# Beryl2000/SE-UNet-AirSeg

Hardware: AMD Instinct MI355X
Metric: voxels/sec SE-UNet fwd+bwd, 128^3 patch (higher is better)
Workload: dtype bf16

## Files before the change

### se-unet-airseg_amd/csrc/abi.cpp

```cpp
#include "seunet_common.h"
#include "epilogue.h"
#include "volume.h"
#include "wgrad.h"
#include "../../include/seunet_hip.h"

using namespace seunet;

static inline Dims D(seunet_dims d) { return Dims{d.n, d.d, d.h, d.w}; }
static inline hipStream_t S(seunet_stream_t s) { return reinterpret_cast<hipStream_t>(s); }

static int make_src(int nsrc, const void* const* src, const int* src_c, SrcList& l) {
  SEUNET_CHECK(nsrc >= 1 && nsrc <= 3 && src && src_c, "bad source list");
  l = SrcList{};
  l.n = nsrc;
  for (int i = 0; i < nsrc; ++i) { l.ptr[i] = src[i]; l.C[i] = src_c[i]; }
  return 0;
}

namespace seunet { extern unsigned long long* g_conv_debug; }

extern "C" {

int seunet_debug_set_buffer(void* p) { seunet::g_conv_debug = reinterpret_cast<unsigned long long*>(p); return 0; }
int seunet_debug_upsample2_form(int dtype, int c, seunet_dims dims, int backward) { return upsample2_form(dtype, c, D(dims), backward != 0); }
// ... 236 lines not shown
                         seunet_stream_t s) {
  SEUNET_CHECK(side && out && scale >= 1, "side_upsample: bad argument");
  return launch_side_upsample(side, c, scale, out, c_total, c_off, D(low), S(s));
}

int seunet_head_fwd(const float* const* level_maps, int nlevels, const float* bias, float* pred, seunet_dims d, seunet_stream_t s) {
  SEUNET_CHECK(level_maps && bias && pred, "head_fwd: null tensor");
  return launch_head_fwd(level_maps, nlevels, bias, pred, D(d), S(s));
}
size_t seunet_head_bwd_tmp_floats(seunet_dims d) { return head_bwd_tmp_floats(D(d)); }
int seunet_head_bwd(const float* g_pred, float* const* g_levels, int nlevels, float* tmp, float* g_bias, seunet_dims d,
                    seunet_stream_t s) {
  SEUNET_CHECK(g_pred && g_levels && tmp, "head_bwd: null tensor");
  return launch_head_bwd(g_pred, g_levels, nlevels, tmp, g_bias, D(d), S(s));
}

int seunet_loss_partial_floats(void) { return loss_partials() * SEUNET_LOSS_NSUMS; }
int seunet_loss_sums(const float* pred, int apply_sigmoid, const float* target, const float* weight, const float* skel,
                     long long n, float* partial, double* sums, int terms, seunet_stream_t s) {
  SEUNET_CHECK(pred && target && partial && sums && n >= 1, "loss_sums: bad argument");
  SEUNET_CHECK(terms >= 0 && terms <= 7, "loss_sums: terms=%d is not a mask of SEUNET_LOSS_DICE | _GUL | _ATR", terms);
  return launch_loss_sums(pred, apply_sigmoid, target, weight, skel, n, partial, sums, S(s), terms);
}
int seunet_loss_value(const double* sums0, double c_dice0, double c_gul0, double c_atr0, const double* sums1, double c_dice1,
                      double c_gul1, double c_atr1, float* value, seunet_stream_t s) {
  SEUNET_CHECK(sums0 && value, "loss_value: null argument");
  return launch_loss_value(sums0, c_dice0, c_gul0, c_atr0, sums1, c_dice1, c_gul1, c_atr1, value, S(s));
}
int seunet_loss_grad(const float* pred, int apply_sigmoid, const float* target, const float* weight, const float* skel,
                     long long n, const double* sums, float c_dice, float c_gul, float c_atr, float g_scale,
// ... 413 lines not shown
```

### se-unet-airseg_amd/csrc/heads.hip

```cpp
#include "seunet_common.h"
#include "trilinear.h"

namespace seunet {

__global__ void side_upsample_kernel(const float* __restrict__ side, int C, int scale,
                                     float* __restrict__ out, int c_total, int c_off, int D, int H, int W,
                                     long long total) {
  const int Do = D * scale, Ho = H * scale, Wo = W * scale;
  const float rz = ac_scale(D, Do), ry = ac_scale(H, Ho), rx = ac_scale(W, Wo);
  const long long Vo = (long long)Do * Ho * Wo;
  for (long long i = blockIdx.x * (long long)blockDim.x + threadIdx.x; i < total;
       i += (long long)gridDim.x * blockDim.x) {
    long long r = i;
    const int xo = (int)(r % Wo); r /= Wo;
    const int yo = (int)(r % Ho); r /= Ho;
    const int zo = (int)(r % Do);
    const long long n = r / Do;
    int z0, z1, y0, y1, x0, x1; float lz, ly, lx;
    ac_src(zo, rz, D, z0, z1, lz);
    ac_src(yo, ry, H, y0, y1, ly);
    ac_src(xo, rx, W, x0, x1, lx);
    for (int c = 0; c < C; ++c) {
      float acc = 0.f;
#pragma unroll
// ... 46 lines not shown
      const float w00 = (1.f - lz) * (1.f - ly), w01 = (1.f - lz) * ly, w10 = lz * (1.f - ly), w11 = lz * ly;
      const float rx = ac_scale(Wl, W);
#pragma unroll
      for (int k = 0; k < 4; ++k) {
        int x0, x1; float lx;
        ac_src(4 * xq + k, rx, Wl, x0, x1, lx);
        const float a0 = w00 * r00[x0] + w01 * r01[x0] + w10 * r10[x0] + w11 * r11[x0];
        const float a1 = w00 * r00[x1] + w01 * r01[x1] + w10 * r10[x1] + w11 * r11[x1];
        acc[k] += (1.f - lx) * a0 + lx * a1;
      }
    }
    *reinterpret_cast<float4*>(pred + o) = make_float4(acc[0], acc[1], acc[2], acc[3]);
  }
}
constexpr int HF_RPW = 4;
__global__ void __launch_bounds__(256)
head_fwd_rows_kernel(HeadLevels lv, const float* __restrict__ bias, float* __restrict__ pred, int D, int H, int W) {
  extern __shared__ float hrow[];
  const int wv = __builtin_amdgcn_readfirstlane(threadIdx.x >> 6), lane = threadIdx.x & 63;
  const int per_row = (W >> 1) + (W >> 2) + (W >> 3);
  float* const rb = hrow + wv * HF_RPW * per_row;
  const float b0 = bias[0];
  const int ybl = (H + 4 * HF_RPW - 1) / (4 * HF_RPW);
  const int yb = blockIdx.x % ybl, zo = (blockIdx.x / ybl) % D, n = blockIdx.x / (ybl * D);
  const int ybase = (yb * 4 + wv) * HF_RPW;
  float2 v0[HF_RPW];
#pragma unroll
  for (int r = 0; r < HF_RPW; ++r) {
    const int yo = ybase + r < H ? ybase + r : H - 1;
    v0[r] = (lv.map[0] && 2 * lane < W) ? *reinterpret_cast<const float2*>(lv.map[0] + (((long long)n * D + zo) * H + yo) * W + 2 * lane)
                                        : make_float2(0.f, 0.f);
  }
  int tx0[3][2], tx1[3][2]; float tlx[3][2];
#pragma unroll
  for (int l = 1; l < 4; ++l)
#pragma unroll
    for (int k = 0; k < 2; ++k) ac_src(2 * lane + k, ac_scale(W >> l, W), W >> l, tx0[l - 1][k], tx1[l - 1][k], tlx[l - 1][k]);
#pragma unroll
  for (int l = 1; l < 4; ++l) {
    if (!lv.map[l]) continue;
    const int Dl = D >> l, Hl = H >> l, Wl = W >> l;
    int z0, z1; float lz;
    ac_src(zo, ac_scale(Dl, D), Dl, z0, z1, lz);
    const float* m = lv.map[l] + (long long)n * Dl * Hl * Wl;
    const int lbase = (l > 1 ? (W >> 1) : 0) + (l > 2 ? (W >> 2) : 0);
#pragma unroll
    for (int r = 0; r < HF_RPW; ++r) {
      const int yo = ybase + r < H ? ybase + r : H - 1;
      int y0, y1; float ly;
      ac_src(yo, ac_scale(Hl, H), Hl, y0, y1, ly);
      const float* r00 = m + (z0 * Hl + y0) * Wl;
      const float* r01 = m + (z0 * Hl + y1) * Wl;
      const float* r10 = m + (z1 * Hl + y0) * Wl;
      const float* r11 = m + (z1 * Hl + y1) * Wl;
      const float w00 = (1.f - lz) * (1.f - ly), w01 = (1.f - lz) * ly, w10 = lz * (1.f - ly), w11 = lz * ly;
      for (int xc = lane; xc < Wl; xc += 64)
        rb[r * per_row + lbase + xc] = w00 * r00[xc] + w01 * r01[xc] + w10 * r10[xc] + w11 * r11[xc];
    }
  }
  __builtin_amdgcn_wave_barrier();
#pragma unroll
  for (int r = 0; r < HF_RPW; ++r) {
    const int yo = ybase + r;
    if (yo >= H) break;
    const long long orow = (((long long)n * D + zo) * H + yo) * W;
    for (int x = 2 * lane; x < W; x += 128) {
      float acc[2] = {b0, b0};
      if (lv.map[0]) {
        const float2 v = x < 128 ? v0[r] : *reinterpret_cast<const float2*>(lv.map[0] + orow + x);
        acc[0] += v.x; acc[1] += v.y;
      }
      int lb = r * per_row;
// ... 3 lines not shown
        const int Wl = W >> l;
#pragma unroll
        for (int k = 0; k < 2; ++k) {
          int x0 = tx0[l - 1][k], x1 = tx1[l - 1][k]; float lx = tlx[l - 1][k];
          if (x >= 128) ac_src(x + k, ac_scale(Wl, W), Wl, x0, x1, lx);
          acc[k] += (1.f - lx) * rb[lb + x0] + lx * rb[lb + x1];
        }
        lb += Wl;
      }
      *reinterpret_cast<float2*>(pred + orow + x) = make_float2(acc[0], acc[1]);
    }
  }
}

constexpr int HB_ROWS = 32, HB_K = 24, HB_PAD = 24, HB_KA = 8;
__global__ void __launch_bounds__(256)
head_bwd_x_multi_kernel(const float* __restrict__ g, float* __restrict__ t1a, float* __restrict__ t1b, float* __restrict__ t1c,
                        int nl, int W, long long rows, double* __restrict__ bias_part) {
  extern __shared__ float hsm[];
  const int RW = W + HB_PAD;
  float* tab = hsm + 4 * RW;
  const int wv = threadIdx.x >> 6, lane = threadIdx.x & 63;
  const long long row0 = (long long)blockIdx.x * HB_ROWS;
  constexpr int RPW = HB_ROWS / 4;
  const bool pf = W <= 256;
  float pre[RPW][4];
  if (pf) {
#pragma unroll
    for (int j = 0; j < RPW; ++j) {
      const long long row = row0 + wv + 4 * j;
#pragma unroll
      for (int k = 0; k < 4; ++k) {
        const int x = lane + 64 * k;
        pre[j][k] = (row < rows && x < W) ? g[row * W + x] : 0.f;
      }
    }
  }
  float* const outs[3] = {t1a, t1b, t1c};
  int ebase[4] = {0, 0, W >> 1, (W >> 1) + (W >> 2)};
  const int nent = (nl > 1 ? W >> 1 : 0) + (nl > 2 ? W >> 2 : 0) + (nl > 3 ? W >> 3 : 0);
  for (int e = threadIdx.x; e < nent; e += 256) {
    const int l = e < ebase[2] ? 1 : (e < ebase[3] ? 2 : 3);
    const int i = e - ebase[l], Wl = W >> l;
    const float rs = ac_scale(Wl, W);
    int lo, hi;
    ac_range(i, rs, W, lo, hi);
    float* t = tab + e * (HB_K + 2);
    int cnt = 0, first = lo;
    bool started = false;
    for (int o = lo; o <= hi; ++o) {
      const float w = ac_weight(o, i, rs, Wl);
      if (!started && w == 0.f) { first = o + 1; continue; }
      started = true;
      if (cnt < HB_K) t[2 + cnt] = w;
      ++cnt;
    }
    t[0] = __int_as_float(first);
    t[1] = __int_as_float(cnt < HB_K ? cnt : HB_K);
  }
  for (int i = threadIdx.x; i < 4 * HB_PAD; i += 256) hsm[(i / HB_PAD) * RW + W + i % HB_PAD] = 0.f;
  __syncthreads();
  const int e0 = lane, e1 = lane + 64;
  float wa[HB_KA], wb[HB_K];
  int fa = 0, fb = 0, ca = 0, cb = 0;
  {
    if (e0 < nent) { const float* t = tab + e0 * (HB_K + 2); fa = __float_as_int(t[0]); ca = __float_as_int(t[1]); }
    if (e1 < nent) { const float* t = tab + e1 * (HB_K + 2); fb = __float_as_int(t[0]); cb = __float_as_int(t[1]); }
#pragma unroll
    for (int k = 0; k < HB_KA; ++k) wa[k] = (e0 < nent && k < ca) ? tab[e0 * (HB_K + 2) + 2 + k] : 0.f;
#pragma unroll
    for (int k = 0; k < HB_K; ++k) wb[k] = (e1 < nent && k < cb) ? tab[e1 * (HB_K + 2) + 2 + k] : 0.f;
  }
  const bool fast = nent <= 128 && __all(ca <= HB_KA && cb <= HB_K && fa + HB_KA <= RW && fb + HB_K <= RW);
  int ka = 0, kb = 0;
#pragma unroll
  for (int off = 32; off >= 1; off >>= 1) { ca = max(ca, shfl_xor_settled(ca, off)); cb = max(cb, shfl_xor_settled(cb, off)); }
  ka = (ca + 3) & ~3; kb = (cb + 3) & ~3;
  const int la = e0 < ebase[2] ? 1 : (e0 < ebase[3] ? 2 : 3), lb = e1 < ebase[2] ? 1 : (e1 < ebase[3] ? 2 : 3);
  float* const outa = e0 < nent ? (la == 1 ? t1a : (la == 2 ? t1b : t1c)) : nullptr;
  float* const outb = e1 < nent ? (lb == 1 ? t1a : (lb == 2 ? t1b : t1c)) : nullptr;
  const int cola = e0 - ebase[la], colb = e1 - ebase[lb], wla = W >> la, wlb = W >> lb;
  double sum = 0.0;
#pragma unroll
  for (int j = 0; j < RPW; ++j) {
    const int rr = wv + 4 * j;
    const long long row = row0 + rr;
    if (row >= rows) break;
    float* rb = hsm + wv * RW;
    if (pf) {
#pragma unroll
      for (int k = 0; k < 4; ++k) {
        const int x = lane + 64 * k;
        if (x < W) { rb[x] = pre[j][k]; sum += (double)pre[j][k]; }
      }
    } else {
      for (int x = lane; x < W; x += 64) { const float v = g[row * W + x]; rb[x] = v; sum += (double)v; }
    }
    __builtin_amdgcn_wave_barrier();
    if (fast) {
      float a0 = 0.f, a1 = 0.f;
#pragma unroll
      for (int k = 0; k < HB_KA; ++k)
        if (k < ka) a0 += wa[k] * rb[fa + k];
#pragma unroll
      for (int k = 0; k < HB_K; ++k)
        if (k < kb) a1 += wb[k] * rb[fb + k];
      if (outa) outa[row * wla + cola] = a0;
      if (outb) outb[row * wlb + colb] = a1;
      __builtin_amdgcn_wave_barrier();
      continue;
    }
    for (int e = lane; e < nent; e += 64) {
      const int l = e < ebase[2] ? 1 : (e < ebase[3] ? 2 : 3);
      float* out = outs[l - 1];
      if (out == nullptr) continue;
      const float* t = tab + e * (HB_K + 2);
      const int first = __float_as_int(t[0]), cnt = __float_as_int(t[1]);
      float acc = 0.f;
      for (int k = 0; k < cnt; k += 4) {
        float w[4], v[4];
#pragma unroll
        for (int j = 0; j < 4; ++j) {
          const bool in = k + j < cnt;
          w[j] = in ? t[2 + k + j] : 0.f;
          v[j] = in ? rb[first + k + j] : 0.f;
        }
#pragma unroll
        for (int j = 0; j < 4; ++j)
          if (w[j] != 0.f) acc += w[j] * v[j];
      }
      out[row * (W >> l) + (e - ebase[l])] = acc;
    }
    __builtin_amdgcn_wave_barrier();
  }
  if (bias_part != nullptr) {
#pragma unroll
    for (int off = 32; off >= 1; off >>= 1) sum += shfl_xor_settled(sum, off);
    __shared__ double wsum[4];
    if (lane == 0) wsum[wv] = sum;
    __syncthreads();
    if (threadIdx.x == 0) bias_part[blockIdx.x] = ((wsum[0] + wsum[1]) + wsum[2]) + wsum[3];
  }
}

__global__ void __launch_bounds__(1024) sum_stage2_wide_kernel(const double* __restrict__ partial, int n, float* __restrict__ out) {
  double s = 0.0;
  for (int i = threadIdx.x; i < n; i += 1024) s += partial[i];
#pragma unroll
  for (int off = 32; off >= 1; off >>= 1) s += shfl_xor_settled(s, off);
  __shared__ double w[16];
  if ((threadIdx.x & 63) == 0) w[threadIdx.x >> 6] = s;
  __syncthreads();
  if (threadIdx.x == 0) {
    double t = 0.0;
    for (int k = 0; k < 16; ++k) t += w[k];
    out[0] = (float)t;
// ... 14 lines not shown
  if (threadIdx.x == 0) {
    double t = 0.0;
    for (int k = 0; k < 16; ++k) t += w[k];
    out[0] = (float)t;
  }
}

int launch_side_upsample(const float* side, int C, int scale, float* out, int c_total, int c_off, Dims dl,
                         hipStream_t s) {
  const long long total = (long long)dl.N * dl.vox() * scale * scale * scale;
  side_upsample_kernel<<<grid_for(total), 256, 0, s>>>(side, C, scale, out, c_total, c_off, dl.D, dl.H, dl.W, total);
  SEUNET_LAUNCH_CHECK();
  return 0;
}

int launch_head_fwd(const float* const* level_maps, int nlevels, const float* bias, float* pred, Dims d0,
                    hipStream_t s) {
  SEUNET_CHECK(nlevels >= 1 && nlevels <= 4, "head: nlevels=%d out of range", nlevels);
  HeadLevels lv;
  for (int l = 0; l < 4; ++l) lv.map[l] = l < nlevels ? level_maps[l] : nullptr;
  for (int l = 1; l < nlevels; ++l)
    SEUNET_CHECK((d0.D >> l) >= 1 && (d0.H >> l) >= 1 && (d0.W >> l) >= 1, "head: volume too small for level %d", l);
  SEUNET_CHECK(d0.W % 4 == 0, "head: W=%d must be a multiple of 4", d0.W);
  if (d0.W % 8 == 0 && d0.W <= 2048 && (long long)d0.D * d0.H * d0.W < (1ll << 31)) {
    const size_t lds = (size_t)4 * HF_RPW * ((d0.W >> 1) + (d0.W >> 2) + (d0.W >> 3)) * sizeof(float);
    const int ybl = (d0.H + 4 * HF_RPW - 1) / (4 * HF_RPW);
    head_fwd_rows_kernel<<<d0.N * d0.D * ybl, 256, lds, s>>>(lv, bias, pred, d0.D, d0.H, d0.W);
  } else {
    const long long total4 = (long long)d0.N * d0.vox() / 4;
    head_fwd_kernel<<<grid_for(total4), 256, 0, s>>>(lv, bias, pred, d0.D, d0.H, d0.W, total4);
  }
  SEUNET_LAUNCH_CHECK();
  return 0;
}

struct AxisJob { const float* in; float* out; int I, O; long long inner, total; };
struct AxisJobs { AxisJob j[3]; int njobs; const double* bias_part; int bias_n; float* g_bias; };
__global__ void __launch_bounds__(256) up_transpose_axis_multi_kernel(AxisJobs jobs) {
  if ((int)blockIdx.y >= jobs.njobs) {
    if (blockIdx.x == 0) sum_stage2_wide_by_256(jobs.bias_part, jobs.bias_n, jobs.g_bias);
    return;
  }
  const AxisJob jb = jobs.j[blockIdx.y];
  if (jb.total == 0) return;
  const float rs = ac_scale(jb.I, jb.O);
  const unsigned inner = (unsigned)jb.inner, I = (unsigned)jb.I, total = (unsigned)jb.total;
  for (unsigned idx = blockIdx.x * blockDim.x + threadIdx.x; idx < total; idx += gridDim.x * blockDim.x) {
    const unsigned q = idx / inner;
    const unsigned in_i = idx - q * inner;
    const unsigned outer = q / I;
    const int i = (int)(q - outer * I);
    int lo, hi;
    ac_range(i, rs, jb.O, lo, hi);
    float acc = 0.f;
    for (int o = lo; o <= hi; o += 4) {
// ... 15 lines not shown
static HeadBwdLayout head_bwd_layout(Dims d0, int nlevels) {
  HeadBwdLayout m{};
  const long long rows = (long long)d0.N * d0.D * d0.H, V = rows * d0.W;
  long long off = 0, off2 = V - V / 8;
  for (int l = 1; l < nlevels; ++l) {
    m.t1[l] = off;
    off += rows * (d0.W >> l);
    m.t2[l] = off2;
    off2 += (long long)d0.N * d0.D * (d0.H >> l) * (d0.W >> l);
  }
  m.part = (V + V / 2 + 64 + 1) & ~1ll;
  m.total = V + V / 2 + 64 + 2 * ((rows + HB_ROWS - 1) / HB_ROWS + 64);
  return m;
}
size_t head_bwd_tmp_floats(Dims d0) { return (size_t)head_bwd_layout(d0, 4).total; }
int launch_head_bwd(const float* g_pred, float* const* g_levels, int nlevels, float* tmp, float* g_bias,
                    Dims d0, hipStream_t s) {
  SEUNET_CHECK(nlevels >= 1 && nlevels <= 4, "head: nlevels=%d out of range", nlevels);
  const long long rows = (long long)d0.N * d0.D * d0.H;
  const long long V = rows * d0.W;
  const HeadBwdLayout m = head_bwd_layout(d0, nlevels);
  float* t1[4] = {nullptr, nullptr, nullptr, nullptr};
  float* t2[4] = {nullptr, nullptr, nullptr, nullptr};
  for (int l = 1; l < nlevels; ++l) {
    if (g_levels[l]) t1[l] = tmp + m.t1[l];
    t2[l] = tmp + m.t2[l];
  }
  double* part = reinterpret_cast<double*>(tmp + m.part);
  const int nblk = (int)((rows + HB_ROWS - 1) / HB_ROWS);
  SEUNET_CHECK(d0.W <= 1024, "head_bwd: W=%d too large", d0.W);
  SEUNET_CHECK(V / 2 < (1ll << 31), "head_bwd: %lld voxels per call exceed the 32-bit index range of the axis passes", V);
  const size_t lds = ((size_t)4 * (d0.W + HB_PAD) + (size_t)(d0.W - (d0.W >> 3)) * (HB_K + 2)) * sizeof(float);
  head_bwd_x_multi_kernel<<<nblk, 256, lds, s>>>(g_pred, t1[1], t1[2], t1[3], nlevels, d0.W, rows, g_bias ? part : nullptr);
  AxisJobs jy{}, jz{};
  long long max_y = 0, max_z = 0;
  int njobs = 0;
  for (int l = 1; l < nlevels; ++l) {
    if (!g_levels[l]) continue;
    const int Dl = d0.D >> l, Hl = d0.H >> l, Wl = d0.W >> l;
    const long long ty = (long long)d0.N * d0.D * Hl * Wl, tz = (long long)d0.N * Dl * Hl * Wl;
    jy.j[njobs] = AxisJob{t1[l], t2[l], Hl, d0.H, (long long)Wl, ty};
    jz.j[njobs] = AxisJob{t2[l], g_levels[l], Dl, d0.D, (long long)Hl * Wl, tz};
    max_y = ty > max_y ? ty : max_y;
    max_z = tz > max_z ? tz : max_z;
    ++njobs;
  }
  jy.njobs = jz.njobs = njobs;
  if (njobs) {
    if (g_bias) { jy.bias_part = part; jy.bias_n = nblk; jy.g_bias = g_bias; }
    up_transpose_axis_multi_kernel<<<dim3((unsigned)grid_for(max_y), (unsigned)njobs + (g_bias ? 1 : 0)), 256, 0, s>>>(jy);
    up_transpose_axis_multi_kernel<<<dim3((unsigned)grid_for(max_z), (unsigned)njobs), 256, 0, s>>>(jz);
  } else if (g_bias) {
    sum_stage2_wide_kernel<<<1, 1024, 0, s>>>(part, nblk, g_bias);
  }
  SEUNET_LAUNCH_CHECK();
  return 0;
}

}
```

### se-unet-airseg_amd/csrc/net.cpp

```cpp
#include "seunet_common.h"
#include "epilogue.h"
#include "wgrad.h"
#include "../../include/seunet_hip.h"

#include <algorithm>
#include <cstdio>
#include <cstring>
#include <string>
#include <vector>

namespace seunet {

ConvKernel wgrad_kernel(int dtype, int taps, int dil, const SrcList& x, int cin_logical, int cout, Dims d, long long src_dist) {
  if (taps == 1) {
    const int combos = cdiv(cin_logical, 32) * cdiv(cout, 32);
    const long long nv = (long long)d.N * d.vox();
    const bool pays = combos >= 16 || (combos >= 8 && nv >= 500000);
    return pays && wgrad_1x1_supported(dtype, x, cin_logical, cout) ? ConvKernel::Wgrad1x1 : ConvKernel::Tiled;
  }
  const bool fine = d.W >= 32 && (long long)d.D * d.H * d.W >= 48LL * 48 * 48;
  const bool pays = fine || dil == 2 || cin_logical >= 256;
  return pays && wgrad_march_supported(dtype, taps, dil, x, cin_logical, cout, d, src_dist) ? ConvKernel::March : ConvKernel::Tiled;
}

// ... 500 lines not shown
    const int t = c.o.src[0];
    mark("pool_fwd:", c.o.name);
    return launch_maxpool_fwd(p.d.dtype, at(p.feat[t]), p.C[t], at(p.feat[c.o.dst]), p.dims_of(t), s);
  }

  int up_forward(const Op& c) {
    const int t = c.o.src[0];
    mark("up_fwd:", c.o.name);
    return launch_upsample2_fwd(p.d.dtype, at(p.feat[t]), p.C[t], at(p.feat[c.o.dst]), p.dims_of(t), s);
  }

  int heads_forward(float* pred0, float* pred1) {
    float* const pred[2] = {pred0, pred1};
    const Dims d1{1, p.dims[0].D, p.dims[0].H, p.dims[0].W};
    mark("head_fwd");
    for (int h = 0; h < 2; ++h) {
      if (pred[h] == nullptr) continue;
      const int nl = 4 - h;
      if (p.d.n_classes > 1) {
        if (int e = per_sample_class(p.lvl[h], 0, nl, [&](float* const* lm, size_t nc) {
              return launch_head_fwd(lm, nl, par(kG.head_b[h]) + nc % p.d.n_classes, pred[h] + nc * d1.vox(), d1, s);
            })) return e;
      } else {
        const float* lm[4] = {fat(p.lvl[h][0]), fat(p.lvl[h][1]), fat(p.lvl[h][2]), fat(p.lvl[h][3])};
        if (int e = launch_head_fwd(lm, nl, par(kG.head_b[h]), pred[h], p.dims[0], s)) return e;
      }
    }
    mark("outside");
    return 0;
  }

  int forward(const float* x, const float* drop1, const float* drop2, float* pred0, float* pred1) {
    skip_enc_head = pred0 == nullptr;
    drops[0] = drop1; drops[1] = drop2;
    if (int e = pack_all_weights(false)) return e;
    mark("pack_input");
    if (int e = launch_pack_input(p.d.dtype, x, p.d.in_channel, at(p.feat[T_X0]), p.dims[0], s)) return e;
    for (int i = 0; i < kNumOps; ++i) {
      const Op c = op(i);
      const OpKind k = c.o.kind;
      if (int e = k == OP_GATED ? gated_forward(c) : k == OP_CAT ? cat_forward(c) : k == OP_POOL ? pool_forward(c) : up_forward(c))
// ... 38 lines not shown
    gd.n = x.n;
    for (int k = 0; k < x.n; ++k) {
      const int t = o.src[k];
      gd.C[k] = p.C[t];
      gd.ptr[k] = is_input(t) ? nullptr : at(p.grad[t]);
      gd.acc[k] = (!is_input(t) && written[t]) ? 1 : 0;
      if (!is_input(t)) written[t] = true;
    }
    mark("dgrad:", o.name);
    return run_conv(r.dgrad, r.taps, o.dil, gsrc, r.cout, par(c.i, P_CONV1_W), 1, at(r.wp_d), nullptr, gd, nullptr, c.dm);
  }

  int heads_backward() {
    const Dims d1{1, p.dims[0].D, p.dims[0].H, p.dims[0].W};
    mark("head_bwd");
    for (int h = 0; h < 2; ++h) {
      const int nl = 4 - h;
      float* gb = grads[kG.head_b[h]];
      if (p.d.n_classes > 1) {
        if (int e = per_sample_class(p.glvl[h], 1, nl, [&](float* const* gl, size_t nc) {
              return launch_head_bwd(g_pred[h] + nc * d1.vox(), gl, nl, fat(p.head_tmp), fat(p.cls_bias) + nc, d1, s);
            })) return e;
        if (gb)
          if (int e = launch_class_bias_grad(fat(p.cls_bias), p.d.batch, p.d.n_classes, gb, s)) return e;
      } else {
        float* gl[4] = {nullptr, fat(p.glvl[h][1]), fat(p.glvl[h][2]), nl == 4 ? fat(p.glvl[h][3]) : nullptr};
        if (int e = launch_head_bwd(g_pred[h], gl, nl, fat(p.head_tmp), gb, p.dims[0], s)) return e;
      }
    }
    return 0;
  }

  int gated_backward(const Op& c) {
    const OpDesc& o = c.o;
    const int h = kG.head[c.i], P_slots = epi_partials(c.dm);
    const GateBlock blk = gate_block(c);
    SseBwdIn g{written[o.dst] ? at(p.grad[o.dst]) : nullptr, nullptr, c.lv == 0 ? g_pred[h] : fat(p.glvl[h][c.lv])};
    SseHead hd = sse_head(c.i, false);
    float* g_head = head_slice(c.i, grads).gw;
    if (p.d.n_classes > 1) {
      if (int e = level_to_side_grad(c, g.g_level)) return e;
      g.g_level = nullptr;
      g.g_side = fat(p.gside);
// ... 327 lines not shown
```

### se-unet-airseg_amd/csrc/seunet_common.h

```cpp
#pragma once
#include <hip/hip_runtime.h>
#include <stdint.h>
#include <string>

#define SEUNET_F32 0
#define SEUNET_BF16 1
#define SEUNET_F16 2

typedef __bf16 bf16_t;
typedef _Float16 f16_t;

namespace seunet {

void set_error(const std::string& msg);
const char* get_error();
int fail(const char* fmt, ...);
bool prof_on();
void prof_mark(const char* tag, hipStream_t s);

#define SEUNET_CHECK(cond, ...)                       \
  do {                                                \
    if (!(cond)) return ::seunet::fail(__VA_ARGS__);  \
  } while (0)

// ... 276 lines not shown
int launch_adamw(float* const* params, const float* const* grads, float* const* exp_avg, float* const* exp_avg_sq,
                 const long long* counts, int n, double lr, double beta1, double beta2, double eps, double weight_decay,
                 int step, int maximize, hipStream_t s);
int launch_adamw_gated(float* const* params, const float* const* grads, float* const* exp_avg, float* const* exp_avg_sq,
                       const long long* counts, const int* steps, float* const* skipped, int n, double lr, double beta1,
                       double beta2, double eps, double weight_decay, int maximize, const int* flag, float* table, hipStream_t s);
int configure_kernel_lds(unsigned long long& mask, const void* fn, int bytes);
const void* device_zero_page();
int launch_side_upsample(const float* side, int C, int scale, float* out_ncdhw, int c_total,
                         int c_off, Dims dlow, hipStream_t s);
int launch_head_fwd(const float* const* level_maps, int nlevels, const float* bias, float* pred,
                    Dims d0, hipStream_t s);
int launch_head_bwd(const float* g_pred, float* const* g_levels, int nlevels, float* tmp,
                    float* g_bias, Dims d0, hipStream_t s);
size_t head_bwd_tmp_floats(Dims d0);

#define SEUNET_LOSS_NSUMS 7
int loss_partials();
int launch_loss_sums(const float* pred, int apply_sigmoid, const float* target,
                     const float* weight, const float* skel, long long n, float* partial,
                     double* sums, hipStream_t s, int terms = 7);
int launch_loss_value(const double* sums0, double c_dice0, double c_gul0, double c_atr0, const double* sums1, double c_dice1,
                      double c_gul1, double c_atr1, float* value, hipStream_t s);
int launch_loss_grad(const float* pred, int apply_sigmoid, const float* target,
                     const float* weight, const float* skel, long long n, const double* sums,
                     float c_dice, float c_gul, float c_atr, float g_scale,
                     const float* g_scale_dev, float* g_pred, hipStream_t s);
int loss_sample_partials(int batch);
int launch_loss_sums_per_sample(const float* pred, int apply_sigmoid, const float* target, const float* weight, const float* skel,
                                int batch, long long n, float* partial, double* sums, int terms, hipStream_t s);
// ... 14 lines not shown
```

Measured before the change: 590.7 million.

## Batch both deep-supervision heads into shared fwd/bwd launches with plane-level bwd kernel

Forward head kernel now takes both heads via blockIdx.y and preloads the first 64 columns of each low-res source row into registers before the LDS writes. Backward replaces the x-pass plus per-axis transpose launches with one per-plane kernel that does the x and y interpolation in LDS for both heads, followed by a single z-axis launch. The aim is fewer kernel launches and less temporary global traffic for the head gradients. The cost is large LDS use and a fallback path for shapes that don't fit.

```diff
diff --git a/se-unet-airseg_amd/csrc/abi.cpp b/se-unet-airseg_amd/csrc/abi.cpp
--- a/se-unet-airseg_amd/csrc/abi.cpp
+++ b/se-unet-airseg_amd/csrc/abi.cpp
@@ -274,6 +274,25 @@
   SEUNET_CHECK(g_pred && g_levels && tmp, "head_bwd: null tensor");
   return launch_head_bwd(g_pred, g_levels, nlevels, tmp, g_bias, D(d), S(s));
 }
+int seunet_debug_heads_fused(int on) { return set_heads_fused(on != 0) ? 1 : 0; }
+int seunet_debug_head_bwd_plan(seunet_dims d, int nlevels, long long* out) {
+  const HeadPlaneLayout m = head_plane_layout(D(d), nlevels);
+  const long long v[8] = {m.t2[1], m.t2[2], m.t2[3], m.part, m.nparts, m.end, m.stride, (long long)head_bwd_tmp_floats(D(d))};
+  if (out) for (int i = 0; i < 8; ++i) out[i] = v[i];
+  return head_bwd_planes_ok(D(d)) ? 1 : 0;
+}
+int seunet_debug_heads_fwd(const float* const* maps0, int nlevels0, const float* bias0, float* pred0, const float* const* maps1,
+                           int nlevels1, const float* bias1, float* pred1, seunet_dims d, seunet_stream_t s) {
+  SEUNET_CHECK(maps1 && bias1 && pred1 && (!pred0 || (maps0 && bias0)), "heads_fwd: null tensor");
+  const HeadFwdJob hd[2] = {{maps0, nlevels0, bias0, pred0}, {maps1, nlevels1, bias1, pred1}};
+  return pred0 ? launch_heads_fwd(hd, 2, D(d), S(s)) : launch_heads_fwd(hd + 1, 1, D(d), S(s));
+}
+int seunet_debug_heads_bwd(const float* g_pred0, float* const* g_levels0, int nlevels0, float* g_bias0, const float* g_pred1,
+                           float* const* g_levels1, int nlevels1, float* g_bias1, float* tmp, seunet_dims d, seunet_stream_t s) {
+  SEUNET_CHECK(g_pred1 && g_levels1 && tmp && (!g_pred0 || g_levels0), "heads_bwd: null tensor");
+  const HeadBwdJob hd[2] = {{g_pred0, g_levels0, nlevels0, g_bias0}, {g_pred1, g_levels1, nlevels1, g_bias1}};
+  return g_pred0 ? launch_heads_bwd(hd, 2, tmp, D(d), S(s)) : launch_heads_bwd(hd + 1, 1, tmp, D(d), S(s));
+}
 
 int seunet_loss_partial_floats(void) { return loss_partials() * SEUNET_LOSS_NSUMS; }
 int seunet_loss_sums(const float* pred, int apply_sigmoid, const float* target, const float* weight, const float* skel,
diff --git a/se-unet-airseg_amd/csrc/heads.hip b/se-unet-airseg_amd/csrc/heads.hip
--- a/se-unet-airseg_amd/csrc/heads.hip
+++ b/se-unet-airseg_amd/csrc/heads.hip
@@ -84,13 +84,17 @@
   }
 }
 constexpr int HF_RPW = 4;
+struct HeadFwdRow { HeadLevels lv; const float* bias; float* pred; };
+struct HeadFwdRows { HeadFwdRow h[2]; };
 __global__ void __launch_bounds__(256)
-head_fwd_rows_kernel(HeadLevels lv, const float* __restrict__ bias, float* __restrict__ pred, int D, int H, int W) {
+head_fwd_rows_kernel(HeadFwdRows heads, int D, int H, int W) {
   extern __shared__ float hrow[];
+  const HeadLevels lv = heads.h[blockIdx.y].lv;
+  float* const pred = heads.h[blockIdx.y].pred;
   const int wv = __builtin_amdgcn_readfirstlane(threadIdx.x >> 6), lane = threadIdx.x & 63;
   const int per_row = (W >> 1) + (W >> 2) + (W >> 3);
   float* const rb = hrow + wv * HF_RPW * per_row;
-  const float b0 = bias[0];
+  const float b0 = heads.h[blockIdx.y].bias[0];
   const int ybl = (H + 4 * HF_RPW - 1) / (4 * HF_RPW);
   const int yb = blockIdx.x % ybl, zo = (blockIdx.x / ybl) % D, n = blockIdx.x / (ybl * D);
   const int ybase = (yb * 4 + wv) * HF_RPW;
@@ -101,31 +105,49 @@
     v0[r] = (lv.map[0] && 2 * lane < W) ? *reinterpret_cast<const float2*>(lv.map[0] + (((long long)n * D + zo) * H + yo) * W + 2 * lane)
                                         : make_float2(0.f, 0.f);
   }
-  int tx0[3][2], tx1[3][2]; float tlx[3][2];
-#pragma unroll
-  for (int l = 1; l < 4; ++l)
-#pragma unroll
-    for (int k = 0; k < 2; ++k) ac_src(2 * lane + k, ac_scale(W >> l, W), W >> l, tx0[l - 1][k], tx1[l - 1][k], tlx[l - 1][k]);
-#pragma unroll
-  for (int l = 1; l < 4; ++l) {
-    if (!lv.map[l]) continue;
+  struct Src { const float* r00; const float* r01; const float* r10; const float* r11; float w00, w01, w10, w11; };
+  auto src_rows = [&](int l, int r) {
     const int Dl = D >> l, Hl = H >> l, Wl = W >> l;
     int z0, z1; float lz;
     ac_src(zo, ac_scale(Dl, D), Dl, z0, z1, lz);
     const float* m = lv.map[l] + (long long)n * Dl * Hl * Wl;
+    const int yo = ybase + r < H ? ybase + r : H - 1;
+    int y0, y1; float ly;
+    ac_src(yo, ac_scale(Hl, H), Hl, y0, y1, ly);
+    return Src{m + (z0 * Hl + y0) * Wl, m + (z0 * Hl + y1) * Wl, m + (z1 * Hl + y0) * Wl, m + (z1 * Hl + y1) * Wl,
+               (1.f - lz) * (1.f - ly), (1.f - lz) * ly, lz * (1.f - ly), lz * ly};
+  };
+  float c[3][HF_RPW][4];
+#pragma unroll
+  for (int l = 1; l < 4; ++l) {
+#pragma unroll
+    for (int r = 0; r < HF_RPW; ++r) {
+      const bool on = lv.map[l] && lane < (W >> l);
+      Src sr{};
+      if (lv.map[l]) sr = src_rows(l, r);
+      c[l - 1][r][0] = on ? sr.r00[lane] : 0.f;
+      c[l - 1][r][1] = on ? sr.r01[lane] : 0.f;
+      c[l - 1][r][2] = on ? sr.r10[lane] : 0.f;
+      c[l - 1][r][3] = on ? sr.r11[lane] : 0.f;
+    }
+  }
+  int tx0[3][2], tx1[3][2]; float tlx[3][2];
+#pragma unroll
+  for (int l = 1; l < 4; ++l)
+#pragma unroll
+    for (int k = 0; k < 2; ++k) ac_src(2 * lane + k, ac_scale(W >> l, W), W >> l, tx0[l - 1][k], tx1[l - 1][k], tlx[l - 1][k]);
+#pragma unroll
+  for (int l = 1; l < 4; ++l) {
+    if (!lv.map[l]) continue;
+    const int Wl = W >> l;
     const int lbase = (l > 1 ? (W >> 1) : 0) + (l > 2 ? (W >> 2) : 0);
 #pragma unroll
     for (int r = 0; r < HF_RPW; ++r) {
-      const int yo = ybase + r < H ? ybase + r : H - 1;
-      int y0, y1; float ly;
-      ac_src(yo, ac_scale(Hl, H), Hl, y0, y1, ly);
-      const float* r00 = m + (z0 * Hl + y0) * Wl;
-      const float* r01 = m + (z0 * Hl + y1) * Wl;
-      const float* r10 = m + (z1 * Hl + y0) * Wl;
-      const float* r11 = m + (z1 * Hl + y1) * Wl;
-      const float w00 = (1.f - lz) * (1.f - ly), w01 = (1.f - lz) * ly, w10 = lz * (1.f - ly), w11 = lz * ly;
-      for (int xc = lane; xc < Wl; xc += 64)
-        rb[r * per_row + lbase + xc] = w00 * r00[xc] + w01 * r01[xc] + w10 * r10[xc] + w11 * r11[xc];
+      const Src sr = src_rows(l, r);
+      const float* q = c[l - 1][r];
+      if (lane < Wl) rb[r * per_row + lbase + lane] = sr.w00 * q[0] + sr.w01 * q[1] + sr.w10 * q[2] + sr.w11 * q[3];
+      for (int xc = lane + 64; xc < Wl; xc += 64)
+        rb[r * per_row + lbase + xc] = sr.w00 * sr.r00[xc] + sr.w01 * sr.r01[xc] + sr.w10 * sr.r10[xc] + sr.w11 * sr.r11[xc];
     }
   }
   __builtin_amdgcn_wave_barrier();
@@ -159,6 +181,91 @@
 }
 
 constexpr int HB_ROWS = 32, HB_K = 24, HB_PAD = 24, HB_KA = 8;
+
+struct HbEntries {
+  int b2, b3, nent;
+  __device__ __forceinline__ int level(int e) const { return e < b2 ? 1 : (e < b3 ? 2 : 3); }
+  __device__ __forceinline__ int base(int l) const { return l == 1 ? 0 : (l == 2 ? b2 : b3); }
+};
+__device__ __forceinline__ HbEntries hb_entries(int nl, int W) {
+  return HbEntries{W >> 1, (W >> 1) + (W >> 2), (nl > 1 ? W >> 1 : 0) + (nl > 2 ? W >> 2 : 0) + (nl > 3 ? W >> 3 : 0)};
+}
+__device__ __forceinline__ void hb_build_table(float* hsm, float* tab, const HbEntries& en, int W, int nrows, int nthreads) {
+  const int RW = W + HB_PAD;
+  for (int e = threadIdx.x; e < en.nent; e += nthreads) {
+    const int l = en.level(e);
+    const int i = e - en.base(l), Wl = W >> l;
+    const float rs = ac_scale(Wl, W);
+    int lo, hi;
+    ac_range(i, rs, W, lo, hi);
+    float* t = tab + e * (HB_K + 2);
+    int cnt = 0, first = lo;
+    bool started = false;
+    for (int o = lo; o <= hi; ++o) {
+      const float w = ac_weight(o, i, rs, Wl);
+      if (!started && w == 0.f) { first = o + 1; continue; }
+      started = true;
+      if (cnt < HB_K) t[2 + cnt] = w;
+      ++cnt;
+    }
+    t[0] = __int_as_float(first);
+    t[1] = __int_as_float(cnt < HB_K ? cnt : HB_K);
+  }
+  for (int i = threadIdx.x; i < nrows * HB_PAD; i += nthreads) hsm[(i / HB_PAD) * RW + W + i % HB_PAD] = 0.f;
+}
+struct HbLaneTaps {
+  float wa[HB_KA], wb[HB_K];
+  int fa, fb, ka, kb;
+  int la, lb, cola, colb;
+  bool fast;
+};
+__device__ __forceinline__ HbLaneTaps hb_lane_taps(const float* tab, const HbEntries& en, int RW, int lane) {
+  HbLaneTaps tp;
+  const int nent = en.nent, e0 = lane, e1 = lane + 64;
+  int ca = 0, cb = 0;
+  tp.fa = tp.fb = 0;
+  if (e0 < nent) { const float* t = tab + e0 * (HB_K + 2); tp.fa = __float_as_int(t[0]); ca = __float_as_int(t[1]); }
+  if (e1 < nent) { const float* t = tab + e1 * (HB_K + 2); tp.fb = __float_as_int(t[0]); cb = __float_as_int(t[1]); }
+#pragma unroll
+  for (int k = 0; k < HB_KA; ++k) tp.wa[k] = (e0 < nent && k < ca) ? tab[e0 * (HB_K + 2) + 2 + k] : 0.f;
+#pragma unroll
+  for (int k = 0; k < HB_K; ++k) tp.wb[k] = (e1 < nent && k < cb) ? tab[e1 * (HB_K + 2) + 2 + k] : 0.f;
+  tp.fast = nent <= 128 && __all(ca <= HB_KA && cb <= HB_K && tp.fa + HB_KA <= RW && tp.fb + HB_K <= RW);
+#pragma unroll
+  for (int off = 32; off >= 1; off >>= 1) { ca = max(ca, shfl_xor_settled(ca, off)); cb = max(cb, shfl_xor_settled(cb, off)); }
+  tp.ka = (ca + 3) & ~3; tp.kb = (cb + 3) & ~3;
+  const int la = en.level(e0), lb = en.level(e1);
+  tp.la = e0 < nent ? la : 0; tp.lb = e1 < nent ? lb : 0;
+  tp.cola = e0 - en.base(la); tp.colb = e1 - en.base(lb);
+  return tp;
+}
+__device__ __forceinline__ void hb_fast_sums(const HbLaneTaps& tp, const float* rb, float& a0, float& a1) {
+  a0 = 0.f; a1 = 0.f;
+#pragma unroll
+  for (int k = 0; k < HB_KA; ++k)
+    if (k < tp.ka) a0 += tp.wa[k] * rb[tp.fa + k];
+#pragma unroll
+  for (int k = 0; k < HB_K; ++k)
+    if (k < tp.kb) a1 += tp.wb[k] * rb[tp.fb + k];
+}
+__device__ __forceinline__ float hb_entry_sum(const float* t, const float* rb) {
+  const int first = __float_as_int(t[0]), cnt = __float_as_int(t[1]);
+  float acc = 0.f;
+  for (int k = 0; k < cnt; k += 4) {
+    float w[4], v[4];
+#pragma unroll
+    for (int j = 0; j < 4; ++j) {
+      const bool in = k + j < cnt;
+      w[j] = in ? t[2 + k + j] : 0.f;
+      v[j] = in ? rb[first + k + j] : 0.f;
+    }
+#pragma unroll
+    for (int j = 0; j < 4; ++j)
+      if (w[j] != 0.f) acc += w[j] * v[j];
+  }
+  return acc;
+}
+
 __global__ void __launch_bounds__(256)
 head_bwd_x_multi_kernel(const float* __restrict__ g, float* __restrict__ t1a, float* __restrict__ t1b, float* __restrict__ t1c,
                         int nl, int W, long long rows, double* __restrict__ bias_part) {
@@ -182,49 +289,14 @@
     }
   }
   float* const outs[3] = {t1a, t1b, t1c};
-  int ebase[4] = {0, 0, W >> 1, (W >> 1) + (W >> 2)};
-  const int nent = (nl > 1 ? W >> 1 : 0) + (nl > 2 ? W >> 2 : 0) + (nl > 3 ? W >> 3 : 0);
-  for (int e = threadIdx.x; e < nent; e += 256) {
-    const int l = e < ebase[2] ? 1 : (e < ebase[3] ? 2 : 3);
-    const int i = e - ebase[l], Wl = W >> l;
-    const float rs = ac_scale(Wl, W);
-    int lo, hi;
-    ac_range(i, rs, W, lo, hi);
-    float* t = tab + e * (HB_K + 2);
-    int cnt = 0, first = lo;
-    bool started = false;
-    for (int o = lo; o <= hi; ++o) {
-      const float w = ac_weight(o, i, rs, Wl);
-      if (!started && w == 0.f) { first = o + 1; continue; }
-      started = true;
-      if (cnt < HB_K) t[2 + cnt] = w;
-      ++cnt;
-    }
-    t[0] = __int_as_float(first);
-    t[1] = __int_as_float(cnt < HB_K ? cnt : HB_K);
-  }
-  for (int i = threadIdx.x; i < 4 * HB_PAD; i += 256) hsm[(i / HB_PAD) * RW + W + i % HB_PAD] = 0.f;
+  const HbEntries en = hb_entries(nl, W);
+  const int nent = en.nent;
+  hb_build_table(hsm, tab, en, W, 4, 256);
   __syncthreads();
-  const int e0 = lane, e1 = lane + 64;
-  float wa[HB_KA], wb[HB_K];
-  int fa = 0, fb = 0, ca = 0, cb = 0;
-  {
-    if (e0 < nent) { const float* t = tab + e0 * (HB_K + 2); fa = __float_as_int(t[0]); ca = __float_as_int(t[1]); }
-    if (e1 < nent) { const float* t = tab + e1 * (HB_K + 2); fb = __float_as_int(t[0]); cb = __float_as_int(t[1]); }
-#pragma unroll
-    for (int k = 0; k < HB_KA; ++k) wa[k] = (e0 < nent && k < ca) ? tab[e0 * (HB_K + 2) + 2 + k] : 0.f;
-#pragma unroll
-    for (int k = 0; k < HB_K; ++k) wb[k] = (e1 < nent && k < cb) ? tab[e1 * (HB_K + 2) + 2 + k] : 0.f;
-  }
-  const bool fast = nent <= 128 && __all(ca <= HB_KA && cb <= HB_K && fa + HB_KA <= RW && fb + HB_K <= RW);
-  int ka = 0, kb = 0;
-#pragma unroll
-  for (int off = 32; off >= 1; off >>= 1) { ca = max(ca, shfl_xor_settled(ca, off)); cb = max(cb, shfl_xor_settled(cb, off)); }
-  ka = (ca + 3) & ~3; kb = (cb + 3) & ~3;
-  const int la = e0 < ebase[2] ? 1 : (e0 < ebase[3] ? 2 : 3), lb = e1 < ebase[2] ? 1 : (e1 < ebase[3] ? 2 : 3);
-  float* const outa = e0 < nent ? (la == 1 ? t1a : (la == 2 ? t1b : t1c)) : nullptr;
-  float* const outb = e1 < nent ? (lb == 1 ? t1a : (lb == 2 ? t1b : t1c)) : nullptr;
-  const int cola = e0 - ebase[la], colb = e1 - ebase[lb], wla = W >> la, wlb = W >> lb;
+  const HbLaneTaps tp = hb_lane_taps(tab, en, RW, lane);
+  float* const outa = tp.la == 1 ? t1a : (tp.la == 2 ? t1b : (tp.la == 3 ? t1c : nullptr));
+  float* const outb = tp.lb == 1 ? t1a : (tp.lb == 2 ? t1b : (tp.lb == 3 ? t1c : nullptr));
+  const int cola = tp.cola, colb = tp.colb, wla = W >> tp.la, wlb = W >> tp.lb;
   double sum = 0.0;
 #pragma unroll
   for (int j = 0; j < RPW; ++j) {
@@ -242,39 +314,20 @@
       for (int x = lane; x < W; x += 64) { const float v = g[row * W + x]; rb[x] = v; sum += (double)v; }
     }
     __builtin_amdgcn_wave_barrier();
-    if (fast) {
-      float a0 = 0.f, a1 = 0.f;
-#pragma unroll
-      for (int k = 0; k < HB_KA; ++k)
-        if (k < ka) a0 += wa[k] * rb[fa + k];
-#pragma unroll
-      for (int k = 0; k < HB_K; ++k)
-        if (k < kb) a1 += wb[k] * rb[fb + k];
+    if (tp.fast) {
+      float a0, a1;
+      hb_fast_sums(tp, rb, a0, a1);
       if (outa) outa[row * wla + cola] = a0;
       if (outb) outb[row * wlb + colb] = a1;
       __builtin_amdgcn_wave_barrier();
       continue;
     }
     for (int e = lane; e < nent; e += 64) {
-      const int l = e < ebase[2] ? 1 : (e < ebase[3] ? 2 : 3);
+      const int l = en.level(e);
       float* out = outs[l - 1];
       if (out == nullptr) continue;
-      const float* t = tab + e * (HB_K + 2);
-      const int first = __float_as_int(t[0]), cnt = __float_as_int(t[1]);
-      float acc = 0.f;
-      for (int k = 0; k < cnt; k += 4) {
-        float w[4], v[4];
-#pragma unroll
-        for (int j = 0; j < 4; ++j) {
-          const bool in = k + j < cnt;
-          w[j] = in ? t[2 + k + j] : 0.f;
-          v[j] = in ? rb[first + k + j] : 0.f;
-        }
-#pragma unroll
-        for (int j = 0; j < 4; ++j)
-          if (w[j] != 0.f) acc += w[j] * v[j];
-      }
-      out[row * (W >> l) + (e - ebase[l])] = acc;
+      const float acc = hb_entry_sum(tab + e * (HB_K + 2), rb);
+      out[row * (W >> l) + (e - en.base(l))] = acc;
     }
     __builtin_amdgcn_wave_barrier();
   }
@@ -285,6 +338,104 @@
     if (lane == 0) wsum[wv] = sum;
     __syncthreads();
     if (threadIdx.x == 0) bias_part[blockIdx.x] = ((wsum[0] + wsum[1]) + wsum[2]) + wsum[3];
+  }
+}
+
+constexpr int HP_NW = 8, HP_RPW = HB_ROWS / 4, HP_MAXGROUPS = 32;
+constexpr size_t HP_LDS_BUDGET = 79 * 1024;
+struct HeadPlaneJob { const float* g; float* t2[3]; double* part; int nl; };
+struct HeadPlaneJobs { HeadPlaneJob h[2]; };
+__global__ void __launch_bounds__(HP_NW * 64)
+head_bwd_plane_kernel(HeadPlaneJobs jobs, int H, int W) {
+  extern __shared__ float hsm[];
+  __shared__ double wsum[HP_MAXGROUPS * 4];
+  const HeadPlaneJob jb = jobs.h[blockIdx.y];
+  const int RW = W + HB_PAD;
+  const HbEntries en = hb_entries(jb.nl, W);
+  const int nent = en.nent;
+  float* const tab = hsm + HP_NW * RW;
+  float* const xs = tab + nent * (HB_K + 2);
+  const int wv = __builtin_amdgcn_readfirstlane(threadIdx.x >> 6), lane = threadIdx.x & 63;
+  const int grp = wv >> 2, w4 = wv & 3;
+  const int ngroups = (H + HB_ROWS - 1) / HB_ROWS;
+  const float* const g = jb.g + (long long)blockIdx.x * H * W;
+  float pre[HP_RPW][4];
+  auto request = [&](int first) {
+#pragma unroll
+    for (int j = 0; j < HP_RPW; ++j) {
+      const int r = first + 4 * j;
+#pragma unroll
+      for (int k = 0; k < 4; ++k) {
+        const int x = lane + 64 * k;
+        pre[j][k] = (r < H && x < W) ? g[r * W + x] : 0.f;
+      }
+    }
+  };
+  request(grp * HB_ROWS + w4);
+  hb_build_table(hsm, tab, en, W, HP_NW, HP_NW * 64);
+  __syncthreads();
+  const HbLaneTaps tp = hb_lane_taps(tab, en, RW, lane);
+  float* const rb = hsm + wv * RW;
+  for (int gi = grp; gi < ngroups; gi += HP_NW / 4) {
+    const int first = gi * HB_ROWS + w4;
+    if (gi != grp) request(first);
+    double sum = 0.0;
+#pragma unroll
+    for (int j = 0; j < HP_RPW; ++j) {
+      const int r = first + 4 * j;
+      if (r >= H) break;
+#pragma unroll
+      for (int k = 0; k < 4; ++k) {
+        const int x = lane + 64 * k;
+        if (x < W) { rb[x] = pre[j][k]; sum += (double)pre[j][k]; }
+      }
+      __builtin_amdgcn_wave_barrier();
+      float* const xr = xs + r * nent;
+      if (tp.fast) {
+        float a0, a1;
+        hb_fast_sums(tp, rb, a0, a1);
+        if (tp.la) xr[lane] = a0;
+        if (tp.lb) xr[lane + 64] = a1;
+      } else {
+        for (int e = lane; e < nent; e += 64) xr[e] = hb_entry_sum(tab + e * (HB_K + 2), rb);
+      }
+      __builtin_amdgcn_wave_barrier();
+    }
+#pragma unroll
+    for (int off = 32; off >= 1; off >>= 1) sum += shfl_xor_settled(sum, off);
+    if (lane == 0) wsum[gi * 4 + w4] = sum;
+  }
+  __syncthreads();
+  if (jb.part != nullptr && (int)threadIdx.x < ngroups) {
+    const double* w = wsum + 4 * threadIdx.x;
+    jb.part[(long long)blockIdx.x * ngroups + threadIdx.x] = ((w[0] + w[1]) + w[2]) + w[3];
+  }
+#pragma unroll
+  for (int l = 1; l < 4; ++l) {
+    float* const out = l == 1 ? jb.t2[0] : (l == 2 ? jb.t2[1] : jb.t2[2]);
+    if (l >= jb.nl || out == nullptr) continue;
+    const int Hl = H >> l, Wl = W >> l, nout = Hl * Wl;
+    const float rs = ac_scale(Hl, H);
+    const float* const col = xs + en.base(l);
+    float* const o2 = out + (long long)blockIdx.x * nout;
+    for (int idx = threadIdx.x; idx < nout; idx += HP_NW * 64) {
+      const int i = idx / Wl, xl = idx - i * Wl;
+      int lo, hi;
+      ac_range(i, rs, H, lo, hi);
+      float acc = 0.f;
+      for (int o = lo; o <= hi; o += 4) {
+        float w[4], v[4];
+#pragma unroll
+        for (int k = 0; k < 4; ++k) {
+          w[k] = o + k <= hi ? ac_weight(o + k, i, rs, Hl) : 0.f;
+          v[k] = w[k] != 0.f ? col[(o + k) * nent + xl] : 0.f;
+        }
+#pragma unroll
+        for (int k = 0; k < 4; ++k)
+          if (w[k] != 0.f) acc += w[k] * v[k];
+      }
+      o2[idx] = acc;
+    }
   }
 }
 
@@ -329,31 +480,55 @@
   return 0;
 }
 
-int launch_head_fwd(const float* const* level_maps, int nlevels, const float* bias, float* pred, Dims d0,
-                    hipStream_t s) {
-  SEUNET_CHECK(nlevels >= 1 && nlevels <= 4, "head: nlevels=%d out of range", nlevels);
-  HeadLevels lv;
-  for (int l = 0; l < 4; ++l) lv.map[l] = l < nlevels ? level_maps[l] : nullptr;
-  for (int l = 1; l < nlevels; ++l)
-    SEUNET_CHECK((d0.D >> l) >= 1 && (d0.H >> l) >= 1 && (d0.W >> l) >= 1, "head: volume too small for level %d", l);
+static bool g_heads_fused = true;
+bool set_heads_fused(bool on) { const bool was = g_heads_fused; g_heads_fused = on; return was; }
+
+int launch_heads_fwd(const HeadFwdJob* heads, int nheads, Dims d0, hipStream_t s) {
+  SEUNET_CHECK(nheads >= 1 && nheads <= 2, "heads_fwd: %d heads", nheads);
+  HeadFwdRows rows{};
+  for (int h = 0; h < nheads; ++h) {
+    const int nlevels = heads[h].nlevels;
+    SEUNET_CHECK(nlevels >= 1 && nlevels <= 4, "head: nlevels=%d out of range", nlevels);
+    for (int l = 0; l < 4; ++l) rows.h[h].lv.map[l] = l < nlevels ? heads[h].level_maps[l] : nullptr;
+    for (int l = 1; l < nlevels; ++l)
+      SEUNET_CHECK((d0.D >> l) >= 1 && (d0.H >> l) >= 1 && (d0.W >> l) >= 1, "head: volume too small for level %d", l);
+    rows.h[h].bias = heads[h].bias;
+    rows.h[h].pred = heads[h].pred;
+  }
   SEUNET_CHECK(d0.W % 4 == 0, "head: W=%d must be a multiple of 4", d0.W);
   if (d0.W % 8 == 0 && d0.W <= 2048 && (long long)d0.D * d0.H * d0.W < (1ll << 31)) {
     const size_t lds = (size_t)4 * HF_RPW * ((d0.W >> 1) + (d0.W >> 2) + (d0.W >> 3)) * sizeof(float);
     const int ybl = (d0.H + 4 * HF_RPW - 1) / (4 * HF_RPW);
-    head_fwd_rows_kernel<<<d0.N * d0.D * ybl, 256, lds, s>>>(lv, bias, pred, d0.D, d0.H, d0.W);
+    if (g_heads_fused) {
+      head_fwd_rows_kernel<<<dim3((unsigned)(d0.N * d0.D * ybl), (unsigned)nheads), 256, lds, s>>>(rows, d0.D, d0.H, d0.W);
+    } else {
+      for (int h = 0; h < nheads; ++h) {
+        HeadFwdRows one{};
+        one.h[0] = rows.h[h];
+        head_fwd_rows_kernel<<<dim3((unsigned)(d0.N * d0.D * ybl), 1), 256, lds, s>>>(one, d0.D, d0.H, d0.W);
+      }
+    }
   } else {
     const long long total4 = (long long)d0.N * d0.vox() / 4;
-    head_fwd_kernel<<<grid_for(total4), 256, 0, s>>>(lv, bias, pred, d0.D, d0.H, d0.W, total4);
+    for (int h = 0; h < nheads; ++h)
+      head_fwd_kernel<<<grid_for(total4), 256, 0, s>>>(rows.h[h].lv, rows.h[h].bias, rows.h[h].pred, d0.D, d0.H, d0.W, total4);
   }
   SEUNET_LAUNCH_CHECK();
   return 0;
 }
+int launch_head_fwd(const float* const* level_maps, int nlevels, const float* bias, float* pred, Dims d0,
+                    hipStream_t s) {
+  const HeadFwdJob hd{level_maps, nlevels, bias, pred};
+  return launch_heads_fwd(&hd, 1, d0, s);
+}
 
 struct AxisJob { const float* in; float* out; int I, O; long long inner, total; };
-struct AxisJobs { AxisJob j[3]; int njobs; const double* bias_part; int bias_n; float* g_bias; };
+struct AxisBias { const double* part; int n; float* g_bias; };
+struct AxisJobs { AxisJob j[5]; int njobs; AxisBias bias[2]; };
 __global__ void __launch_bounds__(256) up_transpose_axis_multi_kernel(AxisJobs jobs) {
   if ((int)blockIdx.y >= jobs.njobs) {
-    if (blockIdx.x == 0) sum_stage2_wide_by_256(jobs.bias_part, jobs.bias_n, jobs.g_bias);
+    const AxisBias b = jobs.bias[(int)blockIdx.y - jobs.njobs];
+    if (blockIdx.x == 0) sum_stage2_wide_by_256(b.part, b.n, b.g_bias);
     return;
   }
   const AxisJob jb = jobs.j[blockIdx.y];
@@ -399,9 +574,8 @@
   return m;
 }
 size_t head_bwd_tmp_floats(Dims d0) { return (size_t)head_bwd_layout(d0, 4).total; }
-int launch_head_bwd(const float* g_pred, float* const* g_levels, int nlevels, float* tmp, float* g_bias,
-                    Dims d0, hipStream_t s) {
-  SEUNET_CHECK(nlevels >= 1 && nlevels <= 4, "head: nlevels=%d out of range", nlevels);
+static int head_bwd_three_launches(const float* g_pred, float* const* g_levels, int nlevels, float* tmp, float* g_bias,
+                                   Dims d0, hipStream_t s) {
   const long long rows = (long long)d0.N * d0.D * d0.H;
   const long long V = rows * d0.W;
   const HeadBwdLayout m = head_bwd_layout(d0, nlevels);
@@ -432,7 +606,7 @@
   }
   jy.njobs = jz.njobs = njobs;
   if (njobs) {
-    if (g_bias) { jy.bias_part = part; jy.bias_n = nblk; jy.g_bias = g_bias; }
+    if (g_bias) jy.bias[0] = AxisBias{part, nblk, g_bias};
     up_transpose_axis_multi_kernel<<<dim3((unsigned)grid_for(max_y), (unsigned)njobs + (g_bias ? 1 : 0)), 256, 0, s>>>(jy);
     up_transpose_axis_multi_kernel<<<dim3((unsigned)grid_for(max_z), (unsigned)njobs), 256, 0, s>>>(jz);
   } else if (g_bias) {
@@ -442,4 +616,75 @@
   return 0;
 }
 
-}
+static size_t head_plane_lds(Dims d0) {
+  const size_t nent = (size_t)(d0.W >> 1) + (d0.W >> 2) + (d0.W >> 3);
+  return ((size_t)HP_NW * (d0.W + HB_PAD) + nent * (HB_K + 2) + (size_t)d0.H * nent) * sizeof(float);
+}
+HeadPlaneLayout head_plane_layout(Dims d0, int nlevels) {
+  HeadPlaneLayout m{};
+  long long off = 0;
+  for (int l = 1; l < nlevels; ++l) {
+    m.t2[l] = off;
+    off += (long long)d0.N * d0.D * (d0.H >> l) * (d0.W >> l);
+  }
+  m.part = (off + 1) & ~1ll;
+  m.nparts = (long long)d0.N * d0.D * ((d0.H + HB_ROWS - 1) / HB_ROWS);
+  m.end = m.part + 2 * m.nparts;
+  m.stride = (head_bwd_layout(d0, 4).total / 2) & ~1ll;
+  return m;
+}
+bool head_bwd_planes_ok(Dims d0) {
+  if (d0.W > 256 || d0.H > HB_ROWS * HP_MAXGROUPS) return false;
+  if (head_plane_lds(d0) > HP_LDS_BUDGET) return false;
+  const HeadPlaneLayout m = head_plane_layout(d0, 4);
+  return m.end <= m.stride && (long long)d0.N * d0.D * d0.H * d0.W / 2 < (1ll << 31);
+}
+
+int launch_heads_bwd(const HeadBwdJob* heads, int nheads, float* tmp, Dims d0, hipStream_t s) {
+  SEUNET_CHECK(nheads >= 1 && nheads <= 2, "heads_bwd: %d heads", nheads);
+  for (int h = 0; h < nheads; ++h)
+    SEUNET_CHECK(heads[h].nlevels >= 1 && heads[h].nlevels <= 4, "head: nlevels=%d out of range", heads[h].nlevels);
+  if (!g_heads_fused || !head_bwd_planes_ok(d0)) {
+    for (int h = 0; h < nheads; ++h)
+      if (int e = head_bwd_three_launches(heads[h].g_pred, heads[h].g_levels, heads[h].nlevels, tmp, heads[h].g_bias, d0, s)) return e;
+    return 0;
+  }
+  HeadPlaneJobs pj{};
+  AxisJobs jz{};
+  long long max_z = 0;
+  int nbias = 0;
+  for (int h = 0; h < nheads; ++h) {
+    const HeadBwdJob& hd = heads[h];
+    const HeadPlaneLayout m = head_plane_layout(d0, hd.nlevels);
+    float* const base = tmp + h * m.stride;
+    HeadPlaneJob& j = pj.h[h];
+    j.g = hd.g_pred;
+    j.nl = hd.nlevels;
+    j.part = hd.g_bias ? reinterpret_cast<double*>(base + m.part) : nullptr;
+    for (int l = 1; l < hd.nlevels; ++l) {
+      if (!hd.g_levels[l]) continue;
+      j.t2[l - 1] = base + m.t2[l];
+      const int Dl = d0.D >> l, Hl = d0.H >> l, Wl = d0.W >> l;
+      const long long tz = (long long)d0.N * Dl * Hl * Wl;
+      jz.j[jz.njobs++] = AxisJob{j.t2[l - 1], hd.g_levels[l], Dl, d0.D, (long long)Hl * Wl, tz};
+      max_z = tz > max_z ? tz : max_z;
+    }
+    if (hd.g_bias) jz.bias[nbias++] = AxisBias{j.part, (int)m.nparts, hd.g_bias};
+  }
+  static unsigned long long configured = 0;
+  const size_t lds = head_plane_lds(d0);
+  if (int e = configure_kernel_lds(configured, reinterpret_cast<const void*>(&head_bwd_plane_kernel), (int)HP_LDS_BUDGET)) return e;
+  head_bwd_plane_kernel<<<dim3((unsigned)(d0.N * d0.D), (unsigned)nheads), HP_NW * 64, lds, s>>>(pj, d0.H, d0.W);
+  if (jz.njobs + nbias)
+    up_transpose_axis_multi_kernel<<<dim3((unsigned)grid_for(max_z), (unsigned)(jz.njobs + nbias)), 256, 0, s>>>(jz);
+  SEUNET_LAUNCH_CHECK();
+  return 0;
+}
+
+int launch_head_bwd(const float* g_pred, float* const* g_levels, int nlevels, float* tmp, float* g_bias,
+                    Dims d0, hipStream_t s) {
+  const HeadBwdJob hd{g_pred, g_levels, nlevels, g_bias};
+  return launch_heads_bwd(&hd, 1, tmp, d0, s);
+}
+
+}
diff --git a/se-unet-airseg_amd/csrc/net.cpp b/se-unet-airseg_amd/csrc/net.cpp
--- a/se-unet-airseg_amd/csrc/net.cpp
+++ b/se-unet-airseg_amd/csrc/net.cpp
@@ -538,17 +538,26 @@
     float* const pred[2] = {pred0, pred1};
     const Dims d1{1, p.dims[0].D, p.dims[0].H, p.dims[0].W};
     mark("head_fwd");
-    for (int h = 0; h < 2; ++h) {
-      if (pred[h] == nullptr) continue;
-      const int nl = 4 - h;
-      if (p.d.n_classes > 1) {
+    if (p.d.n_classes > 1) {
+      for (int h = 0; h < 2; ++h) {
+        if (pred[h] == nullptr) continue;
+        const int nl = 4 - h;
         if (int e = per_sample_class(p.lvl[h], 0, nl, [&](float* const* lm, size_t nc) {
               return launch_head_fwd(lm, nl, par(kG.head_b[h]) + nc % p.d.n_classes, pred[h] + nc * d1.vox(), d1, s);
             })) return e;
-      } else {
-        const float* lm[4] = {fat(p.lvl[h][0]), fat(p.lvl[h][1]), fat(p.lvl[h][2]), fat(p.lvl[h][3])};
-        if (int e = launch_head_fwd(lm, nl, par(kG.head_b[h]), pred[h], p.dims[0], s)) return e;
-      }
+      }
+    } else {
+      const float* lm[2][4];
+      HeadFwdJob hd[2];
+      int nh = 0;
+      for (int h = 0; h < 2; ++h) {
+        if (pred[h] == nullptr) continue;
+        for (int l = 0; l < 4; ++l) lm[nh][l] = fat(p.lvl[h][l]);
+        hd[nh] = HeadFwdJob{lm[nh], 4 - h, par(kG.head_b[h]), pred[h]};
+        ++nh;
+      }
+      if (nh)
+        if (int e = launch_heads_fwd(hd, nh, p.dims[0], s)) return e;
     }
     mark("outside");
     return 0;
@@ -617,19 +626,24 @@
   int heads_backward() {
     const Dims d1{1, p.dims[0].D, p.dims[0].H, p.dims[0].W};
     mark("head_bwd");
+    if (p.d.n_classes == 1) {
+      float* gl[2][4];
+      HeadBwdJob hd[2];
+      for (int h = 0; h < 2; ++h) {
+        const int nl = 4 - h;
+        for (int l = 0; l < 4; ++l) gl[h][l] = l >= 1 && l < nl ? fat(p.glvl[h][l]) : nullptr;
+        hd[h] = HeadBwdJob{g_pred[h], gl[h], nl, grads[kG.head_b[h]]};
+      }
+      return launch_heads_bwd(hd, 2, fat(p.head_tmp), p.dims[0], s);
+    }
     for (int h = 0; h < 2; ++h) {
       const int nl = 4 - h;
       float* gb = grads[kG.head_b[h]];
-      if (p.d.n_classes > 1) {
-        if (int e = per_sample_class(p.glvl[h], 1, nl, [&](float* const* gl, size_t nc) {
-              return launch_head_bwd(g_pred[h] + nc * d1.vox(), gl, nl, fat(p.head_tmp), fat(p.cls_bias) + nc, d1, s);
-            })) return e;
-        if (gb)
-          if (int e = launch_class_bias_grad(fat(p.cls_bias), p.d.batch, p.d.n_classes, gb, s)) return e;
-      } else {
-        float* gl[4] = {nullptr, fat(p.glvl[h][1]), fat(p.glvl[h][2]), nl == 4 ? fat(p.glvl[h][3]) : nullptr};
-        if (int e = launch_head_bwd(g_pred[h], gl, nl, fat(p.head_tmp), gb, p.dims[0], s)) return e;
-      }
+      if (int e = per_sample_class(p.glvl[h], 1, nl, [&](float* const* gl, size_t nc) {
+            return launch_head_bwd(g_pred[h] + nc * d1.vox(), gl, nl, fat(p.head_tmp), fat(p.cls_bias) + nc, d1, s);
+          })) return e;
+      if (gb)
+        if (int e = launch_class_bias_grad(fat(p.cls_bias), p.d.batch, p.d.n_classes, gb, s)) return e;
     }
     return 0;
   }
diff --git a/se-unet-airseg_amd/csrc/seunet_common.h b/se-unet-airseg_amd/csrc/seunet_common.h
--- a/se-unet-airseg_amd/csrc/seunet_common.h
+++ b/se-unet-airseg_amd/csrc/seunet_common.h
@@ -314,6 +314,14 @@
 int launch_head_bwd(const float* g_pred, float* const* g_levels, int nlevels, float* tmp,
                     float* g_bias, Dims d0, hipStream_t s);
 size_t head_bwd_tmp_floats(Dims d0);
+struct HeadFwdJob { const float* const* level_maps; int nlevels; const float* bias; float* pred; };
+struct HeadBwdJob { const float* g_pred; float* const* g_levels; int nlevels; float* g_bias; };
+int launch_heads_fwd(const HeadFwdJob* heads, int nheads, Dims d0, hipStream_t s);
+int launch_heads_bwd(const HeadBwdJob* heads, int nheads, float* tmp, Dims d0, hipStream_t s);
+bool head_bwd_planes_ok(Dims d0);
+struct HeadPlaneLayout { long long t2[4], part, nparts, end, stride; };
+HeadPlaneLayout head_plane_layout(Dims d0, int nlevels);
+bool set_heads_fused(bool on);
 
 #define SEUNET_LOSS_NSUMS 7
 int loss_partials();
```

New measurement: 589.9 million, median of 3. About the same (-0.1%).
